# pettni/smooth_feedback

Measured on AMD Instinct MI355X. Metric: QP solves/sec, higher is better.
Workload: dtype f64

## Files before the change

smooth_feedback_amd/csrc/capi_sparse.hip:

```cpp
#include <hip/hip_runtime.h>

#include <algorithm>
#include <chrono>
#include <cstdio>
#include <map>
#include <mutex>
#include <string>
#include <vector>

#include "../../include/sfb.h"
#include "capi_common.h"
#include "qp_sparse_kernel.h"
#include "sparse_plan.h"

struct sfb_sparse_qp_plan {
  sfb::SparsePlanHost host;
  bool pruned = false;
  sfb::SparsePlanHost full;
  std::vector<int32_t> Aorig, Amasked;
  std::mutex mu;
  struct DevCopy {
    int32_t *blob = nullptr, *blob_full = nullptr;
    sfb::SparsePlanDev dev{}, dev_full{};
  };
  std::map<int, DevCopy> per_device;
  struct HostDev {
    std::mutex mu;
    std::pair<char *, size_t> ws{nullptr, 0};
    int64_t batch = -1;
    uint64_t origin = 0;
    hipStream_t stream = nullptr;
    hipEvent_t uploaded = nullptr;
  };
  std::map<int, HostDev> host_dev;
};

namespace sfb {
const SparsePlanHost &plan_host(const sfb_sparse_qp_plan *plan) { return plan->host; }
const SparsePlanHost &plan_io(const sfb_sparse_qp_plan *plan) { return plan->pruned ? plan->full : plan->host; }
}

namespace {

thread_local uint64_t tl_multi_origin = 0;

sfb_status upload_plan(const sfb::SparsePlanHost &h, const std::vector<int32_t> *Aorig, const std::vector<int32_t> *Amasked,
                       int nnzA_io, int32_t **blob_out, sfb::SparsePlanDev &d)
{
  static const std::vector<int32_t> none;
  const std::vector<int32_t> *arrs[] = {&h.Pp, &h.Pi, &h.Pcol, &h.Ap, &h.Aj, &h.Arow, &h.Acp, &h.Aci, &h.Acpos,
                                        &h.Prp, &h.Prj, &h.Prpos, &h.Sp, &h.Sj, &h.Spos, &h.perm, &h.pinv,
                                        &h.Kp, &h.Ki, &h.Kdesc, &h.Lp, &h.Li, &h.Rp, &h.Rk, &h.Rpos, &h.Rlen,
                                        &h.fmap, &h.fidx, &h.bmap, &h.bidx, &h.Kmap, &h.rptr, &h.rtgt, &h.rab, &h.snptr, &h.snR, &h.poff, &h.pmap, &h.fmask, &h.bmask,
                                        &h.f2s, &h.seg, &h.pmapL, &h.rsplit, &h.KmapL, &h.KdescT, &h.KmapT, &h.ztop, &h.ustream, &h.utype, &h.uomap,
                                        Aorig ? Aorig : &none, Amasked ? Amasked : &none};
  constexpr int NA = sizeof(arrs) / sizeof(arrs[0]);
  size_t off[NA + 1];
  off[0] = 0;
  for (int a = 0; a < NA; ++a) off[a + 1] = off[a] + ((arrs[a]->size() + 3) / 4) * 4 + 4;
  const size_t self_words = (sizeof(sfb::SparsePlanDev) + 15) / 16 * 4;
  std::vector<int32_t> blob(off[NA] + self_words, 0);
  for (int a = 0; a < NA; ++a) std::copy(arrs[a]->begin(), arrs[a]->end(), blob.begin() + off[a]);
  int32_t *dblob = nullptr;
  hipError_t e = hipMalloc(reinterpret_cast<void **>(&dblob), blob.size() * sizeof(int32_t));
  if (e != hipSuccess) return sfb::hip_fail(e, "hipMalloc(plan)");
  e = hipMemcpy(dblob, blob.data(), blob.size() * sizeof(int32_t), hipMemcpyHostToDevice);
  if (e != hipSuccess) {
    (void)hipFree(dblob);
    return sfb::hip_fail(e, "hipMemcpy(plan)");
  }
  d.n = h.n; d.m = h.m; d.k = h.k; d.nnzP = h.nnzP; d.nnzA = h.nnzA; d.nnzK = h.nnzK; d.nnzL = h.nnzL;
  const int32_t **ptrs[] = {&d.Pp, &d.Pi, &d.Pcol, &d.Ap, &d.Aj, &d.Arow, &d.Acp, &d.Aci, &d.Acpos,
                            &d.Prp, &d.Prj, &d.Prpos, &d.Sp, &d.Sj, &d.Spos, &d.perm, &d.pinv,
                            &d.Kp, &d.Ki, &d.Kdesc, &d.Lp, &d.Li, &d.Rp, &d.Rk, &d.Rpos, &d.Rlen,
                            &d.fmap, &d.fidx, &d.bmap, &d.bidx, &d.Kmap, &d.rptr, &d.rtgt, &d.rab, &d.snptr, &d.snR, &d.poff, &d.pmap, &d.fmask, &d.bmask,
                            &d.f2s, &d.seg, &d.pmapL, &d.rsplit, &d.KmapL, &d.KdescT, &d.KmapT, &d.ztop, &d.ustream, &d.utype, &d.uomap,
                            &d.Aorig, &d.Amasked};
  d.funits = h.funits; d.bunits = h.bunits; d.ffull0 = h.ffull0; d.ffull1 = h.ffull1; d.bfull0 = h.bfull0; d.bfull1 = h.bfull1; d.idx_scale = h.idx_scale; d.rsteps = h.rsteps; d.maxcol = h.maxcol; d.nsn = h.nsn; d.lds_doubles = h.lds_doubles; d.nseg = h.nseg; d.nnzKT = h.nnzKT; d.nztop = h.nztop; d.units = h.units; d.nunits = h.nunits;
  for (int a = 0; a < NA; ++a) *ptrs[a] = dblob + off[a];
  d.nnzA_io = nnzA_io;
  d.nmasked = Amasked ? (int)Amasked->size() - 512 : 0;
  if (!Aorig) d.Aorig = d.Amasked = nullptr;
  if ((e = sfb::sparse_device_words(&d.dev_active, &d.dev_busy)) != hipSuccess) {
    (void)hipFree(dblob);
    return sfb::hip_fail(e, "launch bookkeeping of the device");
  }
  d.self = reinterpret_cast<const sfb::SparsePlanDev *>(dblob + off[NA]);
  e      = hipMemcpy(dblob + off[NA], &d, sizeof(d), hipMemcpyHostToDevice);
  if (e != hipSuccess) {
    (void)hipFree(dblob);
    return sfb::hip_fail(e, "hipMemcpy(plan struct)");
  }
  *blob_out = dblob;
  return SFB_OK;
}

sfb_status plan_on_device(sfb_sparse_qp_plan *plan, const sfb_sparse_qp_plan::DevCopy **out)
{
  int devid = 0;
  hipError_t e = hipGetDevice(&devid);
  if (e != hipSuccess) return sfb::hip_fail(e, "hipGetDevice");
  std::lock_guard<std::mutex> lk(plan->mu);
  auto it = plan->per_device.find(devid);
  if (it != plan->per_device.end()) {
    *out = &it->second;
    return SFB_OK;
  }
  sfb_sparse_qp_plan::DevCopy dc;
  sfb_status st;
  if (plan->pruned) {
    st = upload_plan(plan->host, &plan->Aorig, &plan->Amasked, plan->full.nnzA, &dc.blob, dc.dev);
    if (st != SFB_OK) return st;
    st = upload_plan(plan->full, nullptr, nullptr, plan->full.nnzA, &dc.blob_full, dc.dev_full);
// ... 413 lines not shown
  if (batch == 0) return sfb::require_device();
  const sfb::SparsePlanHost &h = sfb::plan_io(plan);
  const size_t N = (size_t)h.n, M = (size_t)h.m, NP = (size_t)h.nnzP, NA = (size_t)h.nnzA;
  sfb_qp_params prm_call = *prm;
  uint64_t origin = 1469598103934665603ull;
  {
    std::vector<int> d = sfb::device_list();
    for (int v : d) origin = (origin ^ (uint64_t)(uint32_t)v) * 1099511628211ull;
    origin = (origin ^ (uint64_t)batch) * 1099511628211ull;
    if (origin == 0) origin = 1;
    std::sort(d.begin(), d.end());
    if (std::adjacent_find(d.begin(), d.end()) != d.end()) prm_call.reuse_factor = 0;
  }
  prm_call.verbose = 0;
  const sfb_qp_params *const prm_shard = &prm_call;
  const auto t_call = std::chrono::steady_clock::now();
  const sfb_status rs = sfb::run_sharded(batch, [&](int, int64_t b0, int64_t cnt) {
    const size_t o = (size_t)b0;
    tl_multi_origin = origin;
    const sfb_status s1 = sfb_sparse_qp_solve_batch_host(plan, prm_shard, cnt, Px ? Px + o * NP : nullptr, q + o * N, Ax ? Ax + o * NA : nullptr,
                                          l + o * M, u + o * M, warm_x ? warm_x + o * N : nullptr,
                                          warm_y ? warm_y + o * M : nullptr, x + o * N, y + o * M, obj ? obj + o : nullptr,
                                          iter ? iter + o : nullptr, code + o);
    tl_multi_origin = 0;
    return s1;
  });
  if (rs == SFB_OK && prm->verbose)
    sfb::verbose_report("sparse QP batch (sharded over the device list)", batch, h.n, h.m, -1.0,
                        std::chrono::duration<double, std::milli>(std::chrono::steady_clock::now() - t_call).count(), -1.0, code, iter);
  return rs;
}

}
```

smooth_feedback_amd/csrc/knobs.cpp:

```cpp
#include "knobs.h"

#include <atomic>
#include <cstdio>
#include <cstring>
#include <deque>
#include <map>
#include <mutex>
#include <string>

namespace sfb {

namespace {
const char *const kKnobs[] = {"SFB_SP_GRID",  "SFB_SP_SLICE",  "SFB_SP_PAUSE",      "SFB_SP_PREDICT",   "SFB_SP_LAT",
                              "SFB_SP_FORCE_LAT", "SFB_SP_LAT_WAVES", "SFB_SP_POLISHERS", "SFB_SP_LAT_HELP", "SFB_SP_PHASED", "SFB_SP_LEAN_WAVES", "SFB_MID_GRID", "SFB_MID_SLICE",
                              "SFB_QP4_MAX_WAVES", "SFB_QP_DENSE_BIG", "SFB_EKF_PERSISTENT", "SFB_PLAN_UNITS", "SFB_PLAN_DEBUG", "SFB_MPC_TIMING"};
std::mutex g_mu;
std::atomic<int> g_set{0};
std::map<std::string, const char *> &table()
{
  static std::map<std::string, const char *> t;
  return t;
}
const char *intern(const char *value)
{
  static std::deque<std::string> pool;
  for (const auto &v : pool)
    if (v == value) return v.c_str();
  pool.emplace_back(value);
  return pool.back().c_str();
}
}

const char *knob(const char *name)
{
  if (g_set.load(std::memory_order_acquire) == 0) return nullptr;
  std::lock_guard<std::mutex> lk(g_mu);
  const auto &t = table();
  const auto it = t.find(name);
  return it == t.end() ? nullptr : it->second;
}

int knob_set(const char *name, const char *value)
{
  if (name == nullptr) return 1;
  bool known = false;
  for (const char *k : kKnobs) known = known || std::strcmp(k, name) == 0;
  if (!known) return 1;
  std::lock_guard<std::mutex> lk(g_mu);
// ... 14 lines not shown
```

smooth_feedback_amd/csrc/qp_sparse.hip:

```cpp
#include <hip/hip_runtime.h>

#include <cstdlib>
#include <map>
#include <mutex>

#include <algorithm>
#include <type_traits>
#include <utility>
#include <cfloat>
#include <cmath>

#include "knobs.h"
#include "../../include/sfb.h"
#include "qp_sparse_kernel.h"
#include "wave_util.h"

#ifndef SFB_SWEEP_ASM
#define SFB_SWEEP_ASM 1
#endif
#ifndef SFB_SWEEP_DEPTH
#define SFB_SWEEP_DEPTH 8
#endif

namespace sfb {
// ... 966 lines not shown
    double dv[8];
#pragma unroll
    for (int e = 0; e < 8; ++e) dv[e] = (j0 + e * kWave < k) ? Dinv[j0 + e * kWave] : 0.0;
#pragma unroll
    for (int e = 0; e < 8; ++e)
      if (j0 + e * kWave < k) t[j0 + e * kWave] = dv[e] * t[j0 + e * kWave];
  }
  wave_lds_fence();
  if (next) sweep_dev<8, true, false, true, true>(pl.bidx, uni(pl.bunits), w.LxB, t, lane, pl.bmask, 0, 0, lx, ix, pl.fidx, w.LxF, pl.fmask);
  else sweep_dev<8, true, false, true, false>(pl.bidx, uni(pl.bunits), w.LxB, t, lane, pl.bmask, 0, 0, lx, ix);
}

template<int UB>
__device__ __forceinline__ double lane_max_abs_b(const double *v, const int len, const int lane)
{
  double r = 0.0;
  for (int e0 = lane; e0 < len; e0 += kWave * UB) {
    double x[UB];
#pragma unroll
    for (int e = 0; e < UB; ++e) x[e] = (e0 + e * kWave < len) ? v[e0 + e * kWave] : 0.0;
#pragma unroll
    for (int e = 0; e < UB; ++e) r = fmax(r, fabs(x[e]));
  }
  return wave_max(r);
}
__device__ __forceinline__ double lane_max_abs(const double *v, int len, int lane)
{
  double r = 0.0;
  for (int e = lane; e < len; e += kWave) r = fmax(r, fabs(v[e]));
  return wave_max(r);
}

constexpr int kRowChunk = 8;
template<class PosF, class IdxF>
__device__ __forceinline__ double sp_row_dot(const int p0, const int p1, const double *vals, PosF pos, IdxF idx,
                                             const double *v)
{
  double s = 0.0;
  for (int q = p0; q < p1; q += kRowChunk) {
    int ps[kRowChunk], ix[kRowChunk];
    double a[kRowChunk], x[kRowChunk];
#pragma unroll
    for (int e = 0; e < kRowChunk; ++e) {
      const bool on = q + e < p1;
      ps[e] = on ? pos(q + e) : 0;
      ix[e] = on ? idx(q + e) : 0;
    }
#pragma unroll
    for (int e = 0; e < kRowChunk; ++e) {
      a[e] = vals[ps[e]];
      x[e] = v[ix[e]];
    }
#pragma unroll
    for (int e = 0; e < kRowChunk; ++e)
      if (q + e < p1) s = fma(a[e], x[e], s);
  }
  return s;
}
template<int RB, int CE, class PtrF, class PosF, class IdxF>
__device__ __forceinline__ void sp_rows_dot(double (&s)[RB], const int i0, const int nrows, PtrF ptr, const double *vals, PosF pos,
                                            IdxF idx, const double *v)
{
  int p[RB], pe[RB];
#pragma unroll
  for (int r = 0; r < RB; ++r) {
    const int i = i0 + r * kWave;
    const bool on = i < nrows;
    p[r]  = on ? ptr(i) : 0;
    pe[r] = on ? ptr(i + 1) : 0;
    s[r]  = 0.0;
  }
  for (;;) {
    bool more = false;
#pragma unroll
    for (int r = 0; r < RB; ++r) more = more || p[r] < pe[r];
    if (!more) break;
    int ps[RB][CE], ix[RB][CE];
    double a[RB][CE], x[RB][CE];
#pragma unroll
    for (int r = 0; r < RB; ++r)
#pragma unroll
      for (int e = 0; e < CE; ++e) {
        const bool on = p[r] + e < pe[r];
        ps[r][e] = on ? pos(p[r] + e) : 0;
        ix[r][e] = on ? idx(p[r] + e) : 0;
      }
#pragma unroll
    for (int r = 0; r < RB; ++r)
#pragma unroll
      for (int e = 0; e < CE; ++e) {
        a[r][e] = vals[ps[r][e]];
        x[r][e] = v[ix[r][e]];
      }
#pragma unroll
    for (int r = 0; r < RB; ++r) {
#pragma unroll
      for (int e = 0; e < CE; ++e)
        if (p[r] + e < pe[r]) s[r] = fma(a[r][e], x[r][e], s[r]);
      p[r] += CE;
    }
  }
}
template<int RB, int CE>
__device__ __forceinline__ void sp_rows_A(double (&s)[RB], const SparsePlanDev &pl, const Item &it, int i0, const double *v)
{
  sp_rows_dot<RB, CE>(s, i0, uni(pl.m), [&](int i) { return pl.Ap[i]; }, it.Ax, [](int p) { return p; },
                      [&](int p) { return pl.Aj[p]; }, v);
}
template<int RB, int CE>
__device__ __forceinline__ void sp_rows_P(double (&s)[RB], const SparsePlanDev &pl, const Item &it, int i0, const double *v)
{
  sp_rows_dot<RB, CE>(s, i0, uni(pl.n), [&](int i) { return pl.Prp[i]; }, it.Px, [&](int p) { return pl.Prpos[p]; },
                      [&](int p) { return pl.Prj[p]; }, v);
}
template<int RB, int CE>
__device__ __forceinline__ void sp_rows_At(double (&s)[RB], const SparsePlanDev &pl, const Item &it, int j0, const double *v)
{
  sp_rows_dot<RB, CE>(s, j0, uni(pl.n), [&](int j) { return pl.Acp[j]; }, it.Ax, [&](int p) { return pl.Acpos[p]; },
                      [&](int p) { return pl.Aci[p]; }, v);
}
__device__ __forceinline__ double sp_row_A(const SparsePlanDev &pl, const Item &it, int i, const double *v)
{
  return sp_row_dot(pl.Ap[i], pl.Ap[i + 1], it.Ax, [](int p) { return p; }, [&](int p) { return pl.Aj[p]; }, v);
}
__device__ __forceinline__ double sp_row_At(const SparsePlanDev &pl, const Item &it, int j, const double *v)
{
  return sp_row_dot(pl.Acp[j], pl.Acp[j + 1], it.Ax, [&](int p) { return pl.Acpos[p]; },
                    [&](int p) { return pl.Aci[p]; }, v);
}
__device__ __forceinline__ double sp_row_P(const SparsePlanDev &pl, const Item &it, int i, const double *v)
{
  return sp_row_dot(pl.Prp[i], pl.Prp[i + 1], it.Px, [&](int p) { return pl.Prpos[p]; },
                    [&](int p) { return pl.Prj[p]; }, v);
}

#ifdef SFB_CHECK_FULL_PASSES
constexpr bool kCheckExit = false;
#else
constexpr bool kCheckExit = true;
#endif
#ifdef SFB_PROF_CHECK
enum { kCkChecks, kCkOptimal, kCkDualRes, kCkOrdered, kCkPass2, kCkPinf, kCkPass3, kCkQdx, kCkRows, kCkDinf, kCkCycOpt, kCkCycCert, kCkCycPass2,
       kCkCycPass3, kCkCycTail, kCkHist2 = 16, kCkHist3 = 32, kCkSlots = 48 };
__device__ unsigned long long sfb_check_prof[2][kCkSlots];
constexpr int kStdWavesPerSimd = 2;
#define SFB_CK_ADD(slot, v) { if (lane == 0) atomicAdd(&sfb_check_prof[RBX > 4][slot], (unsigned long long)(v)); }
#define SFB_CK_LAP(slot) { const unsigned now_ = (unsigned)__builtin_amdgcn_s_memtime(); SFB_CK_ADD(slot, now_ - ck_pc) ck_pc = now_; }
#define SFB_CK_ROW(found, hit, base, j0) { if (!found && wave_ballot(hit)) { found = true; SFB_CK_ADD(base + min((j0) / kWave, 14), 1) } }
#define SFB_CK_HIST(base, found) { if (!found) SFB_CK_ADD(base + 15, 1) }
#else
constexpr int kStdWavesPerSimd = 3;
#define SFB_CK_ADD(slot, v)
#define SFB_CK_LAP(slot)
#define SFB_CK_ROW(found, hit, base, j0)
#define SFB_CK_HIST(base, found)
#endif

template<int RBX = 4>
__device__ inline int sp_check_stopping(const SparsePlanDev &pl, const Item &it, const Ws &w,
                                        const DenseKernelParams &kp, double *t, const int lane, float *score = nullptr)
{
  const int n = uni(pl.n), m = uni(pl.m);
  const double inf = INFINITY;
#ifdef SFB_PROF_CHECK
  unsigned ck_pc = (unsigned)__builtin_amdgcn_s_memtime();
  bool ck_first2 = false, ck_first3 = false;
// ... 258 lines not shown
}

__device__ __noinline__ void sp_trace_row(const SparsePlanDev &pl, const Item &it, const Ws &w, double *t, const int lane,
                                          const uint32_t iter, const unsigned long long t0_ticks, double *row)
{
  const int n = uni(pl.n), m = uni(pl.m);
  const int chunk = (uni(pl.k) + 1) / 2;
  double pri = 0.0, dua = 0.0, o = 0.0;
  for (int i = lane; i < m; i += kWave) pri = fmax(pri, fabs(sp_row_A(pl, it, i, w.xus) - w.zus[i]));
  for (int c0 = 0; c0 < n; c0 += chunk) {
    const int c1 = min(n, c0 + chunk);
    for (int j = c0 + lane; j < c1; j += kWave) {
      const double Px = sp_row_P(pl, it, j, w.xus), qj = it.q[j];
      dua = fmax(dua, fabs(Px + qj + sp_row_At(pl, it, j, w.yus)));
      t[2 * (j - c0)]     = 0.5 * Px + qj;
      t[2 * (j - c0) + 1] = w.xus[j];
    }
    wave_sync();
    for (int e = 0; e < c1 - c0; ++e) o += t[2 * e] * t[2 * e + 1];
    wave_sync();
  }
  pri = wave_max(pri);
  dua = wave_max(dua);
  if (lane == 0) {
    row[0] = (double)iter;
    row[1] = o;
    row[2] = pri;
    row[3] = dua;
    row[4] = (double)(wall_clock64() - t0_ticks) * 0.01;
  }
}

template<int RB, int CE, class PtrF, class IdxF, class LoadF, class FmaF>
__device__ __forceinline__ void sp_rows_chain(double (&acc)[RB], const int i0, const int nrows, PtrF ptr, IdxF idx, LoadF load, FmaF fm)
{
  using IdxT = decltype(idx(0));
  using ValT = decltype(load(idx(0)));
  int p[RB], pe[RB];
#pragma unroll
  for (int r = 0; r < RB; ++r) {
    const int i = i0 + r * kWave;
    p[r] = pe[r] = 0;
    if (i < nrows) {
      const auto pp = ptr(i);
      p[r]  = pp.a;
      pe[r] = pp.b;
    }
  }
  IdxT ix[RB][CE];
  auto fetch = [&] {
#pragma unroll
    for (int r = 0; r < RB; ++r)
#pragma unroll
      for (int e = 0; e < CE; ++e) ix[r][e] = idx((p[r] + e < pe[r]) ? p[r] + e : 0);
  };
  fetch();
  for (;;) {
    bool more = false;
#pragma unroll
    for (int r = 0; r < RB; ++r) more = more || p[r] < pe[r];
    if (!more) break;
    ValT v[RB][CE];
    IdxT ic[RB][CE];
    bool on[RB][CE];
#pragma unroll
    for (int r = 0; r < RB; ++r)
#pragma unroll
      for (int e = 0; e < CE; ++e) {
        ic[r][e] = ix[r][e];
        v[r][e]  = load(ic[r][e]);
        on[r][e] = p[r] + e < pe[r];
      }
#pragma unroll
    for (int r = 0; r < RB; ++r) p[r] += CE;
    fetch();
#pragma unroll
    for (int r = 0; r < RB; ++r)
#pragma unroll
      for (int e = 0; e < CE; ++e)
        if (on[r][e]) acc[r] = fm(r, ic[r][e], v[r][e], acc[r]);
  }
}

template<int SD, bool WIDE = false>
__device__ inline void sp_polish(const SparsePlanDev &pl, const Item &it, const Ws &w, const Ws &wf, const DenseKernelParams &kp,
                                 double *t, const double c, const int lane, const bool lean)
{
  const int n = uni(pl.n), m = uni(pl.m), k = uni(pl.k);
  const double inf = INFINITY, eps = DBL_EPSILON;
  for (int i = lane; i < m; i += kWave) {
    const double yi = w.ys[i];
    double a        = 0.0;
    if (yi < -100 * eps && it.l[i] != -inf) a = 1.0;
    if (yi > 100 * eps && it.u[i] != inf) a = 2.0;
    w.act[i] = a;
  }
  for (int e = lane; e < k; e += kWave) w.tv[e] = 0.0;
  wave_sync();
  if (!ldl_numeric_dev<8>(pl, it, wf, t, 1, c, kp.sigma, kp.delta, lane)) return;
  for (uint32_t iter = 0; iter != kp.polish_iter; ++iter) {
#ifndef SFB_POLISH_RB
#define SFB_POLISH_RB 2
#define SFB_POLISH_CE 2
#endif
#ifndef SFB_POLISH_WIDE_RB
#define SFB_POLISH_WIDE_RB 2
#define SFB_POLISH_WIDE_CE 4
#endif
    constexpr int RB = WIDE ? SFB_POLISH_WIDE_RB : SFB_POLISH_RB, CE = WIDE ? SFB_POLISH_WIDE_CE : SFB_POLISH_CE;
    struct Ix { int a, b; };
    struct V3 { double a, b, c; };
    struct V4 { double a, b, c, d; };
    const bool zero_tv = iter == 0;
    for (int i0 = lane; i0 < n; i0 += kWave * RB) {
      double acc[RB], sxi[RB], qi[RB];
      int pv[RB];
#pragma unroll
      for (int r = 0; r < RB; ++r) {
        const int i = i0 + r * kWave;
        const bool on = i < n;
        acc[r] = 0.0;
        sxi[r] = on ? w.sx[i] : 0.0;
        qi[r]  = on ? it.q[i] : 0.0;
        pv[r]  = on ? pl.pinv[i] : k;
      }
      sp_rows_chain<RB, CE>(acc, i0, n, [&](int i) { return zero_tv ? Ix{0, 0} : Ix{pl.Sp[i], pl.Sp[i + 1]}; },
                            [&](int q) { return Ix{pl.Spos[q], pl.Sj[q]}; },
                            [&](const Ix &x) { return V3{it.Px[x.a], w.sx[x.b], w.tv[x.b]}; },
                            [&](int r, const Ix &x, const V3 &v, double a) {
                              const int i = i0 + r * kWave;
                              const double s_ec = (x.b > i) ? v.b : sxi[r], s_er = (x.b > i) ? sxi[r] : v.b;
                              return fma(c * s_ec * s_er * v.a, v.c, a);
                            });
      sp_rows_chain<RB, CE>(acc, i0, n, [&](int i) { return zero_tv ? Ix{0, 0} : Ix{pl.Acp[i], pl.Acp[i + 1]}; },
                            [&](int q) { return Ix{pl.Acpos[q], pl.Aci[q]}; },
                            [&](const Ix &x) { return V4{w.act[x.b], w.sy[x.b], it.Ax[x.a], w.tv[n + x.b]}; },
                            [&](int r, const Ix &, const V4 &v, double a) { return (v.a != 0.0) ? fma(v.b * sxi[r] * v.c, v.d, a) : a; });
#pragma unroll
      for (int r = 0; r < RB; ++r) {
        const double h = -c * (sxi[r] * qi[r]);
        if (i0 + r * kWave < n) t[pv[r]] = h - acc[r];
      }
    }
    for (int r0 = lane; r0 < m; r0 += kWave * RB) {
      double acc[RB], a_[RB], syr[RB], lb[RB], ub[RB];
      int pv[RB];
#pragma unroll
      for (int r = 0; r < RB; ++r) {
        const int rr = r0 + r * kWave;
        const bool on = rr < m;
        acc[r] = 0.0;
        a_[r]  = on ? w.act[rr] : 0.0;
        syr[r] = on ? w.sy[rr] : 0.0;
        lb[r]  = on ? it.l[rr] : 0.0;
        ub[r]  = on ? it.u[rr] : 0.0;
        pv[r]  = on ? pl.pinv[n + rr] : k;
      }
      sp_rows_chain<RB, CE>(acc, r0, m,
                            [&](int rr) { return (!zero_tv && w.act[rr] != 0.0) ? Ix{pl.Ap[rr], pl.Ap[rr + 1]} : Ix{0, 0}; },
                            [&](int q) { return Ix{q, pl.Aj[q]}; },
                            [&](const Ix &x) { return V3{it.Ax[x.a], w.sx[x.b], w.tv[x.b]}; },
                            [&](int r, const Ix &, const V3 &v, double a) { return fma(syr[r] * v.b * v.a, v.c, a); });
#pragma unroll
      for (int r = 0; r < RB; ++r) {
        double h = 0.0;
        if (a_[r] != 0.0) h = (a_[r] == 1.0) ? syr[r] * lb[r] : syr[r] * ub[r];
        if (r0 + r * kWave < m) t[pv[r]] = h - acc[r];
      }
    }
    wave_sync();
    ldl_solve_dev<SD>(pl, wf, t, lane, lean);
    for (int e = lane; e < k; e += kWave) w.tv[e] += t[pl.pinv[e]];
    wave_sync();
  }
  for (int j = lane; j < n; j += kWave) w.xs[j] = w.tv[j];
  for (int i = lane; i < m; i += kWave)
    if (w.act[i] != 0.0) w.ys[i] = w.tv[n + i];
  wave_sync();
}

constexpr int kQFresh = 0, kQHead = 16, kQTail = 32, kQRing = 48;

enum { SP_DONE = 0, SP_SUSPENDED = 2, SP_PAUSED = 3 };

__device__ __forceinline__ bool sp_guard_ok(const SparsePlanDev &pl, const double *__restrict__ Ax, const int lane)
{
  constexpr int UB = 8;
  const int nmasked = uni(pl.nmasked);
  bool bad = false;
  int srcn[UB];
#pragma unroll
  for (int e = 0; e < UB; ++e) srcn[e] = pl.Amasked[lane + e * kWave];
  for (int p0 = lane; p0 < nmasked; p0 += kWave * UB) {
// ... 806 lines not shown
      sp_polish<SFB_SWEEP_DEPTH, WIDE>(pl, it, w, wp, kp, t, c, lane, lean);
    } else {
      if (lane == 0) w.hdr[kHdrStamp] = 0.0;
      sp_polish<SFB_SWEEP_DEPTH, WIDE>(pl, it, w, w, kp, t, c, lane, lean);
    }
  }

  phase_lap(4);
  double *ox = gx + b * (size_t)n, *oy = gy + b * (size_t)m;
  for (int j = lane; j < n; j += kWave) {
    const double v = w.sx[j] * w.xs[j];
    ox[j]    = v;
    w.xus[j] = v;
  }
  for (int i = lane; i < m; i += kWave) oy[i] = w.sy[i] * w.ys[i] / c;
  wave_sync();
  if (gobj != nullptr) {
    const int chunk = (k + 1) / 2;
    double o        = 0.0;
    for (int c0 = 0; c0 < n; c0 += chunk) {
      const int c1 = min(n, c0 + chunk);
      struct Ix { int a, b; };
      struct V2 { double a, b; };
      constexpr int RB = 4, CE = 2;
      for (int i0 = c0 + lane; i0 < c1; i0 += kWave * RB) {
        double acc[RB], xi[RB], qi[RB];
#pragma unroll
        for (int r = 0; r < RB; ++r) {
          const int i = i0 + r * kWave;
          acc[r] = 0.0;
          xi[r]  = (i < c1) ? w.xus[i] : 0.0;
          qi[r]  = (i < c1) ? it.q[i] : 0.0;
        }
        sp_rows_chain<RB, CE>(acc, i0, c1, [&](int i) { return Ix{pl.Prp[i], pl.Prp[i + 1]}; },
                              [&](int q) { return Ix{pl.Prpos[q], pl.Prj[q]}; },
                              [&](const Ix &x) { return V2{it.Px[x.a], w.xus[x.b]}; },
                              [&](int, const Ix &, const V2 &v, double a) { return fma(0.5 * v.a, v.b, a); });
#pragma unroll
        for (int r = 0; r < RB; ++r) {
          const int i = i0 + r * kWave;
          if (i < c1) {
            t[2 * (i - c0)]     = xi[r];
            t[2 * (i - c0) + 1] = acc[r] + qi[r];
          }
        }
      }
      wave_sync();
      const int cnt = c1 - c0;
      int e = 0;
      for (; e + 8 <= cnt; e += 8) {
        vdouble2 v[8];
#pragma unroll
        for (int qq = 0; qq < 8; ++qq) v[qq] = *reinterpret_cast<const vdouble2 *>(t + 2 * (e + qq));
#pragma unroll
        for (int qq = 0; qq < 8; ++qq) o = fma(v[qq].x, v[qq].y, o);
      }
      for (; e < cnt; ++e) o = fma(t[2 * e], t[2 * e + 1], o);
      wave_sync();
    }
    if (lane == 0) gobj[b] = o;
  }
  if (lane == 0) {
    gcode[b] = (ret_code >= 0) ? ret_code : SFB_QP_MAX_ITERATIONS;
    if (giter != nullptr) giter[b] = iter;
#ifdef SFB_SP_TIMELINE
    oy[0] = (double)tl0; oy[1] = (double)tl1; oy[2] = (double)tl2; oy[3] = (double)wall_clock64();
#endif
  }
// ... 572 lines not shown
```

smooth_feedback_amd/csrc/qp_sparse_kernel.h:

```cpp
#pragma once
#include <hip/hip_runtime.h>

#include <cstdint>

#include "qp_dense_kernel.h"

namespace sfb {

#ifndef SFB_KKT_KINDS
#define SFB_KKT_KINDS
enum { K_P = 0, K_A = 1, K_SIGMA = 2, K_RHO = 3 };
#endif

struct SparsePlanDev {
  int n, m, k, nnzP, nnzA, nnzK, nnzL;
  const int32_t *Pp, *Pi, *Pcol, *Ap, *Aj, *Arow;
  const int32_t *Acp, *Aci, *Acpos, *Prp, *Prj, *Prpos, *Sp, *Sj, *Spos;
  const int32_t *perm, *pinv, *Kp, *Ki, *Kdesc, *Lp, *Li, *Rp, *Rk, *Rpos, *Rlen;
  const int32_t *fmap, *fidx, *bmap, *bidx;
  const int32_t *fmask, *bmask;
  int funits, bunits, idx_scale, ffull0, ffull1, bfull0, bfull1;
  const int32_t *Kmap, *rptr, *rtgt, *rab;
  int rsteps, maxcol;
  const int32_t *snptr, *snR, *poff, *pmap;
  int nsn, lds_doubles;
  const int32_t *f2s, *seg, *pmapL, *rsplit, *KmapL, *KdescT, *KmapT, *ztop;
  int nseg, nnzKT, nztop;
  const int32_t *ustream, *utype, *uomap;
  int units, nunits;
  int nnzA_io, nmasked;
  const int32_t *Aorig, *Amasked;
  int32_t *dev_active;
  const unsigned long long *dev_busy;
  const SparsePlanDev *self;
};

hipError_t sparse_device_words(int32_t **active, const unsigned long long **busy);

constexpr int kSweepPadDev = 16;
#ifdef __HIPCC__
#define SFB_HD __host__ __device__
#else
#define SFB_HD
#endif
SFB_HD inline size_t qp_sparse_factor_doubles(int n, int m, int nnzL, int funits, int bunits)
{
  return (size_t)nnzL + 2 * ((size_t)n + m) + 2 + (size_t)(funits + bunits + 2 * kSweepPadDev) * 128;
}
SFB_HD inline size_t qp_sparse_polish_offset(int n, int m, int nnzL, int funits, int bunits, int nnzA_compact)
{
  const size_t k   = (size_t)n + m;
  const size_t off = qp_sparse_factor_doubles(n, m, nnzL, funits, bunits) + k + 6 * (size_t)n + 11 * (size_t)m + 16 +
                     (((size_t)nnzA_compact + 1) & ~(size_t)1);
  return (off + 1) & ~(size_t)1;
}
inline size_t qp_sparse_ws_doubles(int n, int m, int nnzL, int funits, int bunits, int nnzA_compact = 0)
{
  const size_t tot = qp_sparse_polish_offset(n, m, nnzL, funits, bunits, nnzA_compact) +
                     qp_sparse_factor_doubles(n, m, nnzL, funits, bunits) + m + 4;
  return (tot + 1) & ~(size_t)1;
}

inline size_t qp_sparse_ws_doubles(const SparsePlanDev &pl)
{
// ... 14 lines not shown
```

smooth_feedback_amd/csrc/sparse_plan.cpp:

```cpp
#include "knobs.h"
#include "sparse_plan.h"

#include <algorithm>
#include <cstdio>
#include <cstdlib>
#include <iterator>
#include <array>
#include <numeric>
#include <tuple>

namespace sfb {

namespace {

void transpose_pattern(int nouter, int ninner, const std::vector<int32_t> &outer_ptr,
                       const std::vector<int32_t> &inner, std::vector<int32_t> &tp, std::vector<int32_t> &ti,
                       std::vector<int32_t> &tpos)
{
  const int nnz = outer_ptr[nouter];
  tp.assign(ninner + 1, 0);
  ti.resize(nnz);
  tpos.resize(nnz);
  for (int p = 0; p < nnz; ++p) tp[inner[p] + 1]++;
  for (int i = 0; i < ninner; ++i) tp[i + 1] += tp[i];
// ... 186 lines not shown
  for (int step = 0; step < k; ++step) {
    int best = -1;
    for (int a = 0; a < k; ++a) {
      if (done[a]) continue;
      if (best < 0) { best = a; continue; }
      const int sa = stage ? stage[a] : 0, sb = stage ? stage[best] : 0;
      if (sa < sb || (sa == sb && deg[a] < deg[best])) best = a;
    }
    order.push_back(best);
    done[best] = 1;
    nb.clear();
    for (int w = 0; w < W; ++w) {
      uint64_t bits = adj[(size_t)best * W + w];
      while (bits) {
        const int b = (w << 6) + __builtin_ctzll(bits);
        bits &= bits - 1;
        nb.push_back(b);
      }
    }
    for (int a : nb) {
      uint64_t *ra = &adj[(size_t)a * W];
      const uint64_t *rb = &adj[(size_t)best * W];
      for (int w = 0; w < W; ++w) ra[w] |= rb[w];
      ra[a >> 6] &= ~(1ull << (a & 63));
      ra[best >> 6] &= ~(1ull << (best & 63));
    }
    for (int a : nb) deg[a] = degree(a);
  }
  return order;
}

}

bool build_sparse_plan(int n, int m, const int32_t *Pp, const int32_t *Pi, const int32_t *Ap, const int32_t *Aj,
                       int ordering, const int32_t *user_perm, const int32_t *stage, SparsePlanHost &o,
                       const char **msg, int lds_hint)
{
  static const char *ok = "";
  *msg = ok;
  if (n < 1 || m < 1 || !Pp || !Ap) { *msg = "bad sizes / NULL pattern"; return false; }
  const int k = n + m;
  o = SparsePlanHost();
  o.n = n; o.m = m; o.k = k;
  o.nnzP = Pp[n]; o.nnzA = Ap[m];
  if (Pp[0] != 0 || Ap[0] != 0 || o.nnzP < 0 || o.nnzA < 0) { *msg = "pattern pointers must start at 0"; return false; }
  if ((o.nnzP > 0 && !Pi) || (o.nnzA > 0 && !Aj)) { *msg = "NULL index array"; return false; }
  o.Pp.assign(Pp, Pp + n + 1); o.Pi.assign(Pi, Pi + o.nnzP);
  o.Ap.assign(Ap, Ap + m + 1); o.Aj.assign(Aj, Aj + o.nnzA);
  o.Pcol.resize(o.nnzP); o.Arow.resize(o.nnzA);
  for (int c = 0; c < n; ++c) {
    if (Pp[c + 1] < Pp[c]) { *msg = "P column pointers not monotone"; return false; }
    for (int p = Pp[c]; p < Pp[c + 1]; ++p) {
      if (Pi[p] < 0 || Pi[p] >= n) { *msg = "P row index out of range"; return false; }
      if (p > Pp[c] && Pi[p] <= Pi[p - 1]) { *msg = "P row indices must be strictly ascending per column"; return false; }
      o.Pcol[p] = c;
    }
  }
  for (int r = 0; r < m; ++r) {
    if (Ap[r + 1] < Ap[r]) { *msg = "A row pointers not monotone"; return false; }
    for (int p = Ap[r]; p < Ap[r + 1]; ++p) {
      if (Aj[p] < 0 || Aj[p] >= n) { *msg = "A column index out of range"; return false; }
      if (p > Ap[r] && Aj[p] <= Aj[p - 1]) { *msg = "A column indices must be strictly ascending per row"; return false; }
      o.Arow[p] = r;
    }
  }
  transpose_pattern(m, n, o.Ap, o.Aj, o.Acp, o.Aci, o.Acpos);
  transpose_pattern(n, n, o.Pp, o.Pi, o.Prp, o.Prj, o.Prpos);

  {
    o.Sp.assign(n + 1, 0);
    for (int c = 0; c < n; ++c)
      for (int p = Pp[c]; p < Pp[c + 1]; ++p) {
        const int r = Pi[p];
        if (c >= r) { o.Sp[r + 1]++; if (r != c) o.Sp[c + 1]++; }
      }
    for (int i = 0; i < n; ++i) o.Sp[i + 1] += o.Sp[i];
    o.Sj.resize(o.Sp[n]); o.Spos.resize(o.Sp[n]);
    std::vector<int32_t> fill(n, 0);
    for (int c = 0; c < n; ++c)
      for (int p = Pp[c]; p < Pp[c + 1]; ++p)
        if (Pi[p] < c) { o.Sj[o.Sp[c] + fill[c]] = Pi[p]; o.Spos[o.Sp[c] + fill[c]] = p; fill[c]++; }
    for (int c = 0; c < n; ++c)
      for (int p = Pp[c]; p < Pp[c + 1]; ++p) {
        const int r = Pi[p];
        if (c >= r) { o.Sj[o.Sp[r] + fill[r]] = c; o.Spos[o.Sp[r] + fill[r]] = p; fill[r]++; }
      }
  }

  struct Ent { int r, c, kind, idx; };
  std::vector<Ent> ents;
  ents.reserve(o.nnzP + o.nnzA + k);
  std::vector<char> hasdiag(n, 0);
  for (int c = 0; c < n; ++c)
    for (int p = Pp[c]; p < Pp[c + 1]; ++p)
      if (c >= Pi[p]) {
        ents.push_back({Pi[p], c, K_P, p});
        if (Pi[p] == c) hasdiag[c] = 1;
      }
  for (int v = 0; v < n; ++v)
    if (!hasdiag[v]) ents.push_back({v, v, K_SIGMA, v});
// ... 620 lines not shown
      up.lanes = lanes;
      up.sl.clear();
      for (const auto &e : slots[s]) up.sl.push_back({e[1], e[2]});
      const auto cyc = up.place(search_passes);
      cyc_before += cyc.first;
      cyc_after += bank_aware ? cyc.second : cyc.first;
      for (size_t e = 0; e < slots[s].size(); ++e) {
        const int pos  = bank_aware ? up.where[e] : (int)((e % (size_t)lanes) * 2 + e / (size_t)lanes);
        const size_t q = (size_t)s * 128 + (size_t)pos;
        xmap[q] = acc_of(slots[s][e][0]);
        xidx[q] = (slots[s][e][1] * sc) | ((slots[s][e][2] * sc) << 16);
      }
    }
    if (const char *dbg = sfb::knob("SFB_PLAN_DEBUG"); dbg && dbg[0] == '1')
      fprintf(stderr, "[sfb plan] %s sweep: modelled LDS cycles of the slot accesses per sweep: natural placement %ld, bank-aware %ld (floor %d)\n",
              forward ? "forward" : "backward", cyc_before, cyc_after, 16 * steps);
    full0 = full1 = 0;
    for (int s = 0; s < steps;) {
      if ((int)slots[s].size() != cap) { ++s; continue; }
      int e = s;
      while (e < steps && (int)slots[e].size() == cap) ++e;
      const int a = ((s + 7) / 8) * 8, b = (e / 8) * 8;
      if (b - a > full1 - full0) { full0 = a; full1 = b; }
      s = e;
    }
  };
  build(true, o.fmap, o.fidx, o.funits, o.fmask, o.ffull0, o.ffull1);
  build(false, o.bmap, o.bidx, o.bunits, o.bmask, o.bfull0, o.bfull1);

  return true;
}

}
```

smooth_feedback_amd/csrc/sparse_plan.h:

```cpp
#pragma once
#include <cstdint>
#include <vector>

namespace sfb {

#ifndef SFB_KKT_KINDS
#define SFB_KKT_KINDS
enum { K_P = 0, K_A = 1, K_SIGMA = 2, K_RHO = 3 };
#endif

struct SparsePlanHost {
  int n = 0, m = 0, k = 0, nnzP = 0, nnzA = 0, nnzK = 0, nnzL = 0;
  std::vector<int32_t> Pp, Pi, Pcol;
  std::vector<int32_t> Ap, Aj, Arow;
  std::vector<int32_t> Acp, Aci, Acpos;
  std::vector<int32_t> Prp, Prj, Prpos;
  std::vector<int32_t> Sp, Sj, Spos;
  std::vector<int32_t> perm, pinv;
  std::vector<int32_t> Kp, Ki, Kkind, Kidx;
  std::vector<int32_t> Lp, Li;
  std::vector<int32_t> Rp, Rk, Rpos;
  std::vector<int32_t> Rlen;
  static constexpr int kSweepPad = 16;
  std::vector<int32_t> fmap, fidx, bmap, bidx, fmask, bmask;
  int funits = 0, bunits = 0, idx_scale = 1, ffull0 = 0, ffull1 = 0, bfull0 = 0, bfull1 = 0;
  std::vector<int32_t> Kmap, rptr, rtgt, rab, snptr, snR, poff, pmap;
  std::vector<int32_t> Kdesc;
  int rsteps = 0, maxcol = 0, nsn = 0, lds_doubles = 0;
  std::vector<int32_t> f2s;
  static constexpr int kSegStride = 12;
  std::vector<int32_t> seg, pmapL, rsplit, KmapL, KdescT, KmapT, ztop;
  int nseg = 0, nnzKT = 0, nztop = 0;
  std::vector<int32_t> ustream, utype, uomap;
  int units = 0, nunits = 0;
};

bool build_sparse_plan(int n, int m, const int32_t *Pp, const int32_t *Pi, const int32_t *Ap, const int32_t *Aj,
                       int ordering, const int32_t *user_perm, const int32_t *stage, SparsePlanHost &out,
                       const char **msg, int lds_hint = 0);

}
```

Baseline: 224,500.

## Add interleaved ELL-style row views for coalesced sparse row products

```diff
diff --git a/smooth_feedback_amd/csrc/capi_sparse.hip b/smooth_feedback_amd/csrc/capi_sparse.hip
--- a/smooth_feedback_amd/csrc/capi_sparse.hip
+++ b/smooth_feedback_amd/csrc/capi_sparse.hip
@@ -53,7 +53,8 @@
                                         &h.Kp, &h.Ki, &h.Kdesc, &h.Lp, &h.Li, &h.Rp, &h.Rk, &h.Rpos, &h.Rlen,
                                         &h.fmap, &h.fidx, &h.bmap, &h.bidx, &h.Kmap, &h.rptr, &h.rtgt, &h.rab, &h.snptr, &h.snR, &h.poff, &h.pmap, &h.fmask, &h.bmask,
                                         &h.f2s, &h.seg, &h.pmapL, &h.rsplit, &h.KmapL, &h.KdescT, &h.KmapT, &h.ztop, &h.ustream, &h.utype, &h.uomap,
-                                        Aorig ? Aorig : &none, Amasked ? Amasked : &none};
+                                        Aorig ? Aorig : &none, Amasked ? Amasked : &none,
+                                        &h.ArT.rng, &h.ArT.idx, &h.ArT.pos, &h.AcT.rng, &h.AcT.idx, &h.AcT.pos, &h.PrT.rng, &h.PrT.idx, &h.PrT.pos};
   constexpr int NA = sizeof(arrs) / sizeof(arrs[0]);
   size_t off[NA + 1];
   off[0] = 0;
@@ -75,10 +76,12 @@
                             &d.Kp, &d.Ki, &d.Kdesc, &d.Lp, &d.Li, &d.Rp, &d.Rk, &d.Rpos, &d.Rlen,
                             &d.fmap, &d.fidx, &d.bmap, &d.bidx, &d.Kmap, &d.rptr, &d.rtgt, &d.rab, &d.snptr, &d.snR, &d.poff, &d.pmap, &d.fmask, &d.bmask,
                             &d.f2s, &d.seg, &d.pmapL, &d.rsplit, &d.KmapL, &d.KdescT, &d.KmapT, &d.ztop, &d.ustream, &d.utype, &d.uomap,
-                            &d.Aorig, &d.Amasked};
+                            &d.Aorig, &d.Amasked,
+                            &d.ArT, &d.ArTj, &d.ArTpos, &d.AcT, &d.AcTi, &d.AcTpos, &d.PrT, &d.PrTj, &d.PrTpos};
   d.funits = h.funits; d.bunits = h.bunits; d.ffull0 = h.ffull0; d.ffull1 = h.ffull1; d.bfull0 = h.bfull0; d.bfull1 = h.bfull1; d.idx_scale = h.idx_scale; d.rsteps = h.rsteps; d.maxcol = h.maxcol; d.nsn = h.nsn; d.lds_doubles = h.lds_doubles; d.nseg = h.nseg; d.nnzKT = h.nnzKT; d.nztop = h.nztop; d.units = h.units; d.nunits = h.nunits;
   for (int a = 0; a < NA; ++a) *ptrs[a] = dblob + off[a];
   d.nnzA_io = nnzA_io;
+  d.ArStride = h.ArT.stride; d.AcStride = h.AcT.stride; d.PrStride = h.PrT.stride;
   d.nmasked = Amasked ? (int)Amasked->size() - 512 : 0;
   if (!Aorig) d.Aorig = d.Amasked = nullptr;
   if ((e = sfb::sparse_device_words(&d.dev_active, &d.dev_busy)) != hipSuccess) {
@@ -558,3 +561,17 @@
 }
 
 }
+
+extern "C" int sfb_debug_plan_row_view(const sfb_sparse_qp_plan *plan, int which, int32_t *rng, int32_t *idx, int32_t *pos,
+                                       int32_t *stride, int32_t *slots)
+{
+  if (!plan || which < 0 || which > 6 || (which & 3) == 3 || ((which & 4) && !plan->pruned)) return 1;
+  const sfb::SparsePlanHost &h = (which & 4) ? plan->full : plan->host;
+  const sfb::SparsePlanHost::RowView &v = (which & 3) == 0 ? h.ArT : (which & 3) == 1 ? h.AcT : h.PrT;
+  if (stride) *stride = v.stride;
+  if (slots) *slots = v.slots;
+  if (rng) std::copy(v.rng.begin(), v.rng.end(), rng);
+  if (idx) std::copy(v.idx.begin(), v.idx.end(), idx);
+  if (pos) std::copy(v.pos.begin(), v.pos.end(), pos);
+  return 0;
+}
diff --git a/smooth_feedback_amd/csrc/knobs.cpp b/smooth_feedback_amd/csrc/knobs.cpp
--- a/smooth_feedback_amd/csrc/knobs.cpp
+++ b/smooth_feedback_amd/csrc/knobs.cpp
@@ -13,7 +13,7 @@
 namespace {
 const char *const kKnobs[] = {"SFB_SP_GRID",  "SFB_SP_SLICE",  "SFB_SP_PAUSE",      "SFB_SP_PREDICT",   "SFB_SP_LAT",
                               "SFB_SP_FORCE_LAT", "SFB_SP_LAT_WAVES", "SFB_SP_POLISHERS", "SFB_SP_LAT_HELP", "SFB_SP_PHASED", "SFB_SP_LEAN_WAVES", "SFB_MID_GRID", "SFB_MID_SLICE",
-                              "SFB_QP4_MAX_WAVES", "SFB_QP_DENSE_BIG", "SFB_EKF_PERSISTENT", "SFB_PLAN_UNITS", "SFB_PLAN_DEBUG", "SFB_MPC_TIMING"};
+                              "SFB_QP4_MAX_WAVES", "SFB_QP_DENSE_BIG", "SFB_EKF_PERSISTENT", "SFB_PLAN_UNITS", "SFB_PLAN_DEBUG", "SFB_PLAN_ROWT_CAP", "SFB_MPC_TIMING"};
 std::mutex g_mu;
 std::atomic<int> g_set{0};
 std::map<std::string, const char *> &table()
diff --git a/smooth_feedback_amd/csrc/qp_sparse.hip b/smooth_feedback_amd/csrc/qp_sparse.hip
--- a/smooth_feedback_amd/csrc/qp_sparse.hip
+++ b/smooth_feedback_amd/csrc/qp_sparse.hip
@@ -1022,19 +1022,26 @@
 }
 
 constexpr int kRowChunk = 8;
+struct RowRange { int a, b; };
+__device__ __forceinline__ RowRange row_range(const int32_t *rng, const int i)
+{
+  const int2 v = *reinterpret_cast<const int2 *>(rng + 2 * i);
+  return RowRange{v.x, v.y};
+}
 template<class PosF, class IdxF>
-__device__ __forceinline__ double sp_row_dot(const int p0, const int p1, const double *vals, PosF pos, IdxF idx,
+__device__ __forceinline__ double sp_row_dot(const RowRange rg, const int st, const int q0, const double *vals, PosF pos, IdxF idx,
                                              const double *v)
 {
   double s = 0.0;
-  for (int q = p0; q < p1; q += kRowChunk) {
+  int qq = q0;
+  for (int q = rg.a; q < rg.b; q += kRowChunk * st, qq += kRowChunk) {
     int ps[kRowChunk], ix[kRowChunk];
     double a[kRowChunk], x[kRowChunk];
 #pragma unroll
     for (int e = 0; e < kRowChunk; ++e) {
-      const bool on = q + e < p1;
-      ps[e] = on ? pos(q + e) : 0;
-      ix[e] = on ? idx(q + e) : 0;
+      const bool on = q + e * st < rg.b;
+      ps[e] = on ? pos(q + e * st, qq + e) : 0;
+      ix[e] = on ? idx(q + e * st) : 0;
     }
 #pragma unroll
     for (int e = 0; e < kRowChunk; ++e) {
@@ -1043,21 +1050,23 @@
     }
 #pragma unroll
     for (int e = 0; e < kRowChunk; ++e)
-      if (q + e < p1) s = fma(a[e], x[e], s);
+      if (q + e * st < rg.b) s = fma(a[e], x[e], s);
   }
   return s;
 }
-template<int RB, int CE, class PtrF, class PosF, class IdxF>
-__device__ __forceinline__ void sp_rows_dot(double (&s)[RB], const int i0, const int nrows, PtrF ptr, const double *vals, PosF pos,
-                                            IdxF idx, const double *v)
-{
-  int p[RB], pe[RB];
+template<int RB, int CE, class RngF, class BaseF, class PosF, class IdxF>
+__device__ __forceinline__ void sp_rows_dot(double (&s)[RB], const int i0, const int nrows, const int st, RngF rng, BaseF base,
+                                            const double *vals, PosF pos, IdxF idx, const double *v)
+{
+  int p[RB], pe[RB], pq[RB];
 #pragma unroll
   for (int r = 0; r < RB; ++r) {
     const int i = i0 + r * kWave;
     const bool on = i < nrows;
-    p[r]  = on ? ptr(i) : 0;
-    pe[r] = on ? ptr(i + 1) : 0;
+    const RowRange rg = on ? rng(i) : RowRange{0, 0};
+    p[r]  = rg.a;
+    pe[r] = rg.b;
+    pq[r] = on ? base(i) : 0;
     s[r]  = 0.0;
   }
   for (;;) {
@@ -1071,9 +1080,9 @@
     for (int r = 0; r < RB; ++r)
 #pragma unroll
       for (int e = 0; e < CE; ++e) {
-        const bool on = p[r] + e < pe[r];
-        ps[r][e] = on ? pos(p[r] + e) : 0;
-        ix[r][e] = on ? idx(p[r] + e) : 0;
+        const bool on = p[r] + e * st < pe[r];
+        ps[r][e] = on ? pos(p[r] + e * st, pq[r] + e) : 0;
+        ix[r][e] = on ? idx(p[r] + e * st) : 0;
       }
 #pragma unroll
     for (int r = 0; r < RB; ++r)
@@ -1086,42 +1095,44 @@
     for (int r = 0; r < RB; ++r) {
 #pragma unroll
       for (int e = 0; e < CE; ++e)
-        if (p[r] + e < pe[r]) s[r] = fma(a[r][e], x[r][e], s[r]);
-      p[r] += CE;
+        if (p[r] + e * st < pe[r]) s[r] = fma(a[r][e], x[r][e], s[r]);
+      p[r] += CE * st;
+      pq[r] += CE;
     }
   }
 }
 template<int RB, int CE>
 __device__ __forceinline__ void sp_rows_A(double (&s)[RB], const SparsePlanDev &pl, const Item &it, int i0, const double *v)
 {
-  sp_rows_dot<RB, CE>(s, i0, uni(pl.m), [&](int i) { return pl.Ap[i]; }, it.Ax, [](int p) { return p; },
-                      [&](int p) { return pl.Aj[p]; }, v);
+  sp_rows_dot<RB, CE>(s, i0, uni(pl.m), uni(pl.ArStride), [&](int i) { return row_range(pl.ArT, i); }, [&](int i) { return pl.Ap[i]; },
+                      it.Ax, [](int, int q) { return q; }, [&](int p) { return pl.ArTj[p]; }, v);
 }
 template<int RB, int CE>
 __device__ __forceinline__ void sp_rows_P(double (&s)[RB], const SparsePlanDev &pl, const Item &it, int i0, const double *v)
 {
-  sp_rows_dot<RB, CE>(s, i0, uni(pl.n), [&](int i) { return pl.Prp[i]; }, it.Px, [&](int p) { return pl.Prpos[p]; },
-                      [&](int p) { return pl.Prj[p]; }, v);
+  sp_rows_dot<RB, CE>(s, i0, uni(pl.n), uni(pl.PrStride), [&](int i) { return row_range(pl.PrT, i); }, [](int) { return 0; },
+                      it.Px, [&](int p, int) { return pl.PrTpos[p]; }, [&](int p) { return pl.PrTj[p]; }, v);
 }
 template<int RB, int CE>
 __device__ __forceinline__ void sp_rows_At(double (&s)[RB], const SparsePlanDev &pl, const Item &it, int j0, const double *v)
 {
-  sp_rows_dot<RB, CE>(s, j0, uni(pl.n), [&](int j) { return pl.Acp[j]; }, it.Ax, [&](int p) { return pl.Acpos[p]; },
-                      [&](int p) { return pl.Aci[p]; }, v);
+  sp_rows_dot<RB, CE>(s, j0, uni(pl.n), uni(pl.AcStride), [&](int j) { return row_range(pl.AcT, j); }, [](int) { return 0; },
+                      it.Ax, [&](int p, int) { return pl.AcTpos[p]; }, [&](int p) { return pl.AcTi[p]; }, v);
 }
 __device__ __forceinline__ double sp_row_A(const SparsePlanDev &pl, const Item &it, int i, const double *v)
 {
-  return sp_row_dot(pl.Ap[i], pl.Ap[i + 1], it.Ax, [](int p) { return p; }, [&](int p) { return pl.Aj[p]; }, v);
+  return sp_row_dot(row_range(pl.ArT, i), uni(pl.ArStride), pl.Ap[i], it.Ax, [](int, int q) { return q; },
+                    [&](int p) { return pl.ArTj[p]; }, v);
 }
 __device__ __forceinline__ double sp_row_At(const SparsePlanDev &pl, const Item &it, int j, const double *v)
 {
-  return sp_row_dot(pl.Acp[j], pl.Acp[j + 1], it.Ax, [&](int p) { return pl.Acpos[p]; },
-                    [&](int p) { return pl.Aci[p]; }, v);
+  return sp_row_dot(row_range(pl.AcT, j), uni(pl.AcStride), 0, it.Ax, [&](int p, int) { return pl.AcTpos[p]; },
+                    [&](int p) { return pl.AcTi[p]; }, v);
 }
 __device__ __forceinline__ double sp_row_P(const SparsePlanDev &pl, const Item &it, int i, const double *v)
 {
-  return sp_row_dot(pl.Prp[i], pl.Prp[i + 1], it.Px, [&](int p) { return pl.Prpos[p]; },
-                    [&](int p) { return pl.Prj[p]; }, v);
+  return sp_row_dot(row_range(pl.PrT, i), uni(pl.PrStride), 0, it.Px, [&](int p, int) { return pl.PrTpos[p]; },
+                    [&](int p) { return pl.PrTj[p]; }, v);
 }
 
 #ifdef SFB_CHECK_FULL_PASSES
@@ -1446,7 +1457,7 @@
 }
 
 template<int RB, int CE, class PtrF, class IdxF, class LoadF, class FmaF>
-__device__ __forceinline__ void sp_rows_chain(double (&acc)[RB], const int i0, const int nrows, PtrF ptr, IdxF idx, LoadF load, FmaF fm)
+__device__ __forceinline__ void sp_rows_chain(double (&acc)[RB], const int i0, const int nrows, const int st, PtrF ptr, IdxF idx, LoadF load, FmaF fm)
 {
   using IdxT = decltype(idx(0));
   using ValT = decltype(load(idx(0)));
@@ -1466,7 +1477,7 @@
 #pragma unroll
     for (int r = 0; r < RB; ++r)
 #pragma unroll
-      for (int e = 0; e < CE; ++e) ix[r][e] = idx((p[r] + e < pe[r]) ? p[r] + e : 0);
+      for (int e = 0; e < CE; ++e) ix[r][e] = idx((p[r] + e * st < pe[r]) ? p[r] + e * st : 0);
   };
   fetch();
   for (;;) {
@@ -1483,10 +1494,10 @@
       for (int e = 0; e < CE; ++e) {
         ic[r][e] = ix[r][e];
         v[r][e]  = load(ic[r][e]);
-        on[r][e] = p[r] + e < pe[r];
-      }
-#pragma unroll
-    for (int r = 0; r < RB; ++r) p[r] += CE;
+        on[r][e] = p[r] + e * st < pe[r];
+      }
+#pragma unroll
+    for (int r = 0; r < RB; ++r) p[r] += CE * st;
     fetch();
 #pragma unroll
     for (int r = 0; r < RB; ++r)
@@ -1538,7 +1549,7 @@
         qi[r]  = on ? it.q[i] : 0.0;
         pv[r]  = on ? pl.pinv[i] : k;
       }
-      sp_rows_chain<RB, CE>(acc, i0, n, [&](int i) { return zero_tv ? Ix{0, 0} : Ix{pl.Sp[i], pl.Sp[i + 1]}; },
+      sp_rows_chain<RB, CE>(acc, i0, n, 1, [&](int i) { return zero_tv ? Ix{0, 0} : Ix{pl.Sp[i], pl.Sp[i + 1]}; },
                             [&](int q) { return Ix{pl.Spos[q], pl.Sj[q]}; },
                             [&](const Ix &x) { return V3{it.Px[x.a], w.sx[x.b], w.tv[x.b]}; },
                             [&](int r, const Ix &x, const V3 &v, double a) {
@@ -1546,8 +1557,9 @@
                               const double s_ec = (x.b > i) ? v.b : sxi[r], s_er = (x.b > i) ? sxi[r] : v.b;
                               return fma(c * s_ec * s_er * v.a, v.c, a);
                             });
-      sp_rows_chain<RB, CE>(acc, i0, n, [&](int i) { return zero_tv ? Ix{0, 0} : Ix{pl.Acp[i], pl.Acp[i + 1]}; },
-                            [&](int q) { return Ix{pl.Acpos[q], pl.Aci[q]}; },
+      sp_rows_chain<RB, CE>(acc, i0, n, uni(pl.AcStride),
+                            [&](int i) { const RowRange rg = row_range(pl.AcT, i); return zero_tv ? Ix{0, 0} : Ix{rg.a, rg.b}; },
+                            [&](int q) { return Ix{pl.AcTpos[q], pl.AcTi[q]}; },
                             [&](const Ix &x) { return V4{w.act[x.b], w.sy[x.b], it.Ax[x.a], w.tv[n + x.b]}; },
                             [&](int r, const Ix &, const V4 &v, double a) { return (v.a != 0.0) ? fma(v.b * sxi[r] * v.c, v.d, a) : a; });
 #pragma unroll
@@ -1570,9 +1582,9 @@
         ub[r]  = on ? it.u[rr] : 0.0;
         pv[r]  = on ? pl.pinv[n + rr] : k;
       }
-      sp_rows_chain<RB, CE>(acc, r0, m,
-                            [&](int rr) { return (!zero_tv && w.act[rr] != 0.0) ? Ix{pl.Ap[rr], pl.Ap[rr + 1]} : Ix{0, 0}; },
-                            [&](int q) { return Ix{q, pl.Aj[q]}; },
+      sp_rows_chain<RB, CE>(acc, r0, m, uni(pl.ArStride),
+                            [&](int rr) { const RowRange rg = row_range(pl.ArT, rr); return (!zero_tv && w.act[rr] != 0.0) ? Ix{rg.a, rg.b} : Ix{0, 0}; },
+                            [&](int q) { return Ix{pl.ArTpos[q], pl.ArTj[q]}; },
                             [&](const Ix &x) { return V3{it.Ax[x.a], w.sx[x.b], w.tv[x.b]}; },
                             [&](int r, const Ix &, const V3 &v, double a) { return fma(syr[r] * v.b * v.a, v.c, a); });
 #pragma unroll
@@ -2445,8 +2457,8 @@
           xi[r]  = (i < c1) ? w.xus[i] : 0.0;
           qi[r]  = (i < c1) ? it.q[i] : 0.0;
         }
-        sp_rows_chain<RB, CE>(acc, i0, c1, [&](int i) { return Ix{pl.Prp[i], pl.Prp[i + 1]}; },
-                              [&](int q) { return Ix{pl.Prpos[q], pl.Prj[q]}; },
+        sp_rows_chain<RB, CE>(acc, i0, c1, uni(pl.PrStride), [&](int i) { const RowRange rg = row_range(pl.PrT, i); return Ix{rg.a, rg.b}; },
+                              [&](int q) { return Ix{pl.PrTpos[q], pl.PrTj[q]}; },
                               [&](const Ix &x) { return V2{it.Px[x.a], w.xus[x.b]}; },
                               [&](int, const Ix &, const V2 &v, double a) { return fma(0.5 * v.a, v.b, a); });
 #pragma unroll
diff --git a/smooth_feedback_amd/csrc/qp_sparse_kernel.h b/smooth_feedback_amd/csrc/qp_sparse_kernel.h
--- a/smooth_feedback_amd/csrc/qp_sparse_kernel.h
+++ b/smooth_feedback_amd/csrc/qp_sparse_kernel.h
@@ -30,6 +30,8 @@
   int units, nunits;
   int nnzA_io, nmasked;
   const int32_t *Aorig, *Amasked;
+  const int32_t *ArT, *ArTj, *ArTpos, *AcT, *AcTi, *AcTpos, *PrT, *PrTj, *PrTpos;
+  int ArStride, AcStride, PrStride;
   int32_t *dev_active;
   const unsigned long long *dev_busy;
   const SparsePlanDev *self;
diff --git a/smooth_feedback_amd/csrc/sparse_plan.cpp b/smooth_feedback_amd/csrc/sparse_plan.cpp
--- a/smooth_feedback_amd/csrc/sparse_plan.cpp
+++ b/smooth_feedback_amd/csrc/sparse_plan.cpp
@@ -242,6 +242,47 @@
 
 }
 
+void build_row_view(int nrows, const int32_t *ptr, const int32_t *idx, const int32_t *pos, double cap, SparsePlanHost::RowView &out)
+{
+  if (cap < 0.0) {
+    cap = SparsePlanHost::kRowViewCap;
+    if (const char *v = knob("SFB_PLAN_ROWT_CAP")) cap = std::atof(v) / 100.0;
+  }
+  const int nnz = ptr[nrows], nblk = (nrows + 63) / 64;
+  std::vector<int64_t> E(nblk + 1, 0);
+  for (int g = 0; g < nblk; ++g) {
+    int W = 0;
+    for (int i = g * 64; i < std::min(nrows, g * 64 + 64); ++i) W = std::max(W, ptr[i + 1] - ptr[i]);
+    E[g + 1] = E[g] + 64 * (int64_t)W;
+  }
+  out.rng.assign(2 * (size_t)nrows, 0);
+  if ((double)E[nblk] > cap * (double)nnz || E[nblk] > 0x3FFFFFFF) {
+    out.stride = 1;
+    out.slots  = nnz;
+    out.idx.assign(idx, idx + nnz);
+    out.pos.resize(nnz);
+    for (int p = 0; p < nnz; ++p) out.pos[p] = pos ? pos[p] : p;
+    for (int i = 0; i < nrows; ++i) {
+      out.rng[2 * i]     = ptr[i];
+      out.rng[2 * i + 1] = ptr[i + 1];
+    }
+    return;
+  }
+  out.stride = 64;
+  out.slots  = (int)E[nblk];
+  out.idx.assign(out.slots, 0);
+  out.pos.assign(out.slots, 0);
+  for (int i = 0; i < nrows; ++i) {
+    const int first = (int)E[i / 64] + (i & 63), len = ptr[i + 1] - ptr[i];
+    out.rng[2 * i]     = first;
+    out.rng[2 * i + 1] = first + 64 * len;
+    for (int s = 0; s < len; ++s) {
+      out.idx[first + 64 * s] = idx[ptr[i] + s];
+      out.pos[first + 64 * s] = pos ? pos[ptr[i] + s] : ptr[i] + s;
+    }
+  }
+}
+
 bool build_sparse_plan(int n, int m, const int32_t *Pp, const int32_t *Pi, const int32_t *Ap, const int32_t *Aj,
                        int ordering, const int32_t *user_perm, const int32_t *stage, SparsePlanHost &o,
                        const char **msg, int lds_hint)
@@ -276,6 +317,9 @@
   }
   transpose_pattern(m, n, o.Ap, o.Aj, o.Acp, o.Aci, o.Acpos);
   transpose_pattern(n, n, o.Pp, o.Pi, o.Prp, o.Prj, o.Prpos);
+  build_row_view(m, o.Ap.data(), o.Aj.data(), nullptr, -1.0, o.ArT);
+  build_row_view(n, o.Acp.data(), o.Aci.data(), o.Acpos.data(), -1.0, o.AcT);
+  build_row_view(n, o.Prp.data(), o.Prj.data(), o.Prpos.data(), -1.0, o.PrT);
 
   {
     o.Sp.assign(n + 1, 0);
@@ -962,3 +1006,17 @@
 }
 
 }
+
+extern "C" int sfb_debug_row_view(int nrows, const int32_t *ptr, const int32_t *idx, const int32_t *pos, double cap, int64_t room,
+                                  int32_t *rng, int32_t *idx_out, int32_t *pos_out, int32_t *stride, int32_t *slots)
+{
+  sfb::SparsePlanHost::RowView v;
+  sfb::build_row_view(nrows, ptr, idx, pos, cap, v);
+  *stride = v.stride;
+  *slots  = v.slots;
+  if ((int64_t)v.slots > room) return 1;
+  std::copy(v.rng.begin(), v.rng.end(), rng);
+  std::copy(v.idx.begin(), v.idx.end(), idx_out);
+  std::copy(v.pos.begin(), v.pos.end(), pos_out);
+  return 0;
+}
diff --git a/smooth_feedback_amd/csrc/sparse_plan.h b/smooth_feedback_amd/csrc/sparse_plan.h
--- a/smooth_feedback_amd/csrc/sparse_plan.h
+++ b/smooth_feedback_amd/csrc/sparse_plan.h
@@ -33,7 +33,15 @@
   int nseg = 0, nnzKT = 0, nztop = 0;
   std::vector<int32_t> ustream, utype, uomap;
   int units = 0, nunits = 0;
+  struct RowView {
+    std::vector<int32_t> rng, idx, pos;
+    int stride = 1, slots = 0;
+  };
+  static constexpr double kRowViewCap = 2.0;
+  RowView ArT, AcT, PrT;
 };
+
+void build_row_view(int nrows, const int32_t *ptr, const int32_t *idx, const int32_t *pos, double cap, SparsePlanHost::RowView &out);
 
 bool build_sparse_plan(int n, int m, const int32_t *Pp, const int32_t *Pi, const int32_t *Ap, const int32_t *Aj,
                        int ordering, const int32_t *user_perm, const int32_t *stage, SparsePlanHost &out,
```

New measurement: 224,300. No clear change (-0.1%).
